# nipponjo/tts-arabic-pytorch

Hardware: AMD Instinct MI355X
Metric: audio samples/sec (FastPitch+HiFi-GAN, synthetic 64-phoneme inputs) (higher is better)
Workload: dtype f32

## Files before the change

### profiles/launch_classes.py

```python
import csv
import re
import sys
from collections import defaultdict


def classes(path):
    d = defaultdict(lambda: [0, 0])
    other = 0
    with open(path) as f:
        for r in csv.DictReader(f):
            dur = int(r['End_Timestamp']) - int(r['Start_Timestamp'])
            m = re.search(r'conv1d_wino4_f32<(\d+), (\d+), (\d+), (\d+), (\d+), (\d+)>', r['Kernel_Name'])
            if not m:
                other += dur
                continue
            k, noct, nst, epi, lp, pt = map(int, m.groups())
            key = (pt, k, lp, 'residual' if epi == 3 else 'plain', int(r['Grid_Size_X']) // int(r['Workgroup_Size_X']))
            d[key][0] += 1
            d[key][1] += dur
    return d, other


a, oa = classes(sys.argv[1])
b, ob = classes(sys.argv[2])
print(f'{"groups":>6} {"k":>3} {"window":>7} {"epilogue":>9} {"blocks":>7} {"calls":>6} {"us parent":>10} {"us tree":>9} {"ratio":>6}')
ta = tb = 0
for key in sorted(set(a) | set(b), key=lambda t: (-t[0], t[1], t[2], t[3], t[4])):
    ca, da = a.get(key, (0, 0))
    cb, db = b.get(key, (0, 0))
    ta += da
    tb += db
    ua, ub = (da / ca / 1e3 if ca else float('nan')), (db / cb / 1e3 if cb else float('nan'))
    print(f'{"seven" if key[0] == 7 else "six":>6} {key[1]:3d} {"vector" if key[2] == 1 else "strip":>7} {key[3]:>9} {key[4]:7d} {max(ca, cb):6d} '
          f'{ua:10.1f} {ub:9.1f} {ub / ua:6.3f}')
print(f'sum over the conv1d_wino4_f32 launches: {ta / 1e6:.2f} -> {tb / 1e6:.2f} ms; every other kernel: {oa / 1e6:.2f} -> {ob / 1e6:.2f} ms (whole trace)')
```

### tts-arabic-pytorch_amd/csrc/common.hpp

```cpp
#pragma once
#include <hip/hip_runtime.h>
#include <stdint.h>
#include <atomic>
#include <cstdarg>
#include <cstdio>
#include <cstdlib>
#include <string>

#include "../../include/ttsamd.h"

namespace ttsamd {

void set_error(const char* fmt, ...);

#define TTS_CHECK_HIP(expr)                                                         \
    do {                                                                            \
        hipError_t e_ = (expr);                                                     \
        if (e_ != hipSuccess) {                                                     \
            ttsamd::set_error("%s failed: %s (%s:%d)", #expr, hipGetErrorString(e_), \
                              __FILE__, __LINE__);                                  \
            return TTSAMD_EHIP;                                                     \
        }                                                                           \
    } while (0)

// ... 25 lines not shown

#define TTS_OPTIONS(X)                                                                                     \
    X(HIFIGAN_STREAMS, 0, 0, 1)    \
    X(WINO, 0, 0, 1)                                              \
    X(WINO2, 0, 0, 31)             \
    X(WINO4, 0, 0, 127)            \
    X(FUSED_PAIR, 0, 0, 1)                   \
    X(FUSED2, 0, 0, 1)                                           \
    X(FUSED2_MASK, 1, 0, 0x1ff)               \
    X(FUSED2_MASK_N1, 1, 0, 0x1ff)          \
    X(FUSED2_WB, 0, 0, 2)                     \
    X(PAIR4, 0, 0, 2)              \
    X(CONVT, 0, 0, 1)                              \
    X(CONVT_WINO, 0, 0, 2)         \
    X(BFO, 0, 0, 1)                \
    X(BFO_CHAIN, 0, 0, 1)                           \
    X(BFO_CHAIN7, 0, 0, 1)                                 \
    X(BFO_FF, 0, 0, 1)                              \
    X(BFO_SPLITK, 0, 0, 1)                                              \
    X(BFO_SMALL_TILES, 0, 0, 1)            \
    X(BF16_ATTN, 0, 0, 1)                                         \
    X(BF16_PACKED_T, 0, 0, 1)                   \
    X(ATT_RA, 0, 1, 4)                             \
    X(ATT_SPLIT, 0, 0, 1)                      \
    X(XCD_W, 0, 0, 1)                            \
    X(XCD_WMAX_KB, 0, 0, 1 << 20)     \
    X(DEEP_SPLITK, 0, 0, 1)        \
    X(TACO_PERSISTENT, 0, 0, 2)    \
    X(TACO_SEG, 0, 8, 1 << 20)     \
    X(RESBLOCK2_PAIR, 1, 0, 0x3f)
enum Opt : int {
#define TTS_OPT_ENUM(name, kind, lo, hi) OPT_##name,
    TTS_OPTIONS(TTS_OPT_ENUM)
#undef TTS_OPT_ENUM
    OPT_COUNT
};
int64_t opt_int(Opt o, int64_t unset);

struct Arena {
    char* base;
    int64_t size;
    int64_t off = 0;
    bool ok = true;
    Arena(void* p, int64_t n) : base((char*)p), size(n) {}
    template <typename T>
    T* take(int64_t count) {
        int64_t bytes = align_up(count * (int64_t)sizeof(T), 256);
        if (base != nullptr && off + bytes > size) ok = false;
        T* r = base ? (T*)(base + off) : nullptr;
        off += bytes;
        return r;
    }
};

struct ConvParams {
    const float* x;
    int64_t x_bs;
    int32_t x_cs;
    const float* w;
    const void* w_bf16;
    const float* w_wino;
    const float* w_wino4;
    int32_t precision;
    const float* bias;
    float* y;
    int64_t y_bs;
    int32_t y_cs, y_ts;
    const float* res;
    int64_t r_bs;
    int32_t r_cs;
    const int64_t* lens_in;
    const int64_t* lens_out;
    int32_t len_in_mul, len_out_mul;
    int32_t Lin, Nout;
    int32_t Cin, Cout, CoutP, K;
    int32_t dil, pad;
    int32_t n_phase;
    int32_t phase_p;
    float in_slope;
    const float* scale;
    int32_t relu_out;
    int32_t mode;
    float div;
    int32_t batch;
    float* splitk_ws;
    int64_t splitk_floats;
    int32_t ksplit;
    int32_t y_packed;
    float pack_slope;
    int32_t x_packed;
    int32_t xcd_w;
    int32_t tile_major;
    int32_t compact;
    unsigned long long* timing;
    const float* w_wino44;
};
constexpr int64_t kSplitKFloats = 4 << 20;
constexpr int64_t kSplitKFloatsFp = 8 << 20;

void conv_log(const char* kind, int K, int cin, int cout, int nout, int batch, int has_res, int mode, int len_mul, int ragged,
              int n_phase);
bool compact_order(const void* lens, int batch);
int32_t launch_conv(const ConvParams& p, hipStream_t stream);
void note_conv_launch(int32_t route, int32_t ksplit);
void last_conv_launch(int32_t* route, int32_t* ksplit);
bool convt_supported(const ConvParams& p);
int32_t launch_convt(const ConvParams& p, hipStream_t stream);
int32_t launch_upsampler(ConvParams& p, const float* x, const float* w, const void* w_bf16, const float* bias, float* y, int cin, int cout,
                         int u, int kt, int L, int len_mul, float in_slope, bool convt_ok, hipStream_t stream, const float* w_wino = nullptr,
                         const float* bias_wino = nullptr);
bool convt_wino_packable(int cin, int cout, int u);
void pack_convt_wino_weight(const float* w, const float* bias, int cin, int cout, int u, float* out_w, float* out_bias);
bool convt_wino_supported(const ConvParams& p, const float* w_wino, const float* bias_wino);
int32_t launch_convt_wino(const ConvParams& p, const float* w_wino, const float* bias_wino, hipStream_t stream);
bool fused_pair_supported(int32_t channels, int32_t k, int32_t dil, int32_t L, const float* x, const float* y);
int32_t launch_fused_pair(int32_t channels, const float* x, float* y, const float* w1, const float* b1, const float* w2,
                          const float* b2, int32_t k, int32_t dil, const int64_t* lens, int32_t len_mul, int32_t L, int32_t batch,
                          int32_t mode, float div, float slope, hipStream_t stream);
bool fused_pair2_supported(int32_t channels, int32_t k, int32_t dil, int32_t L, const float* x, const float* y, int32_t ntw);
int32_t launch_fused_pair2(int32_t channels, const float* x, float* y, const float* w1, const float* b1, const float* w2,
                           const float* b2, int32_t k, int32_t dil, const int64_t* lens, int32_t len_mul, int32_t L, int32_t batch,
                           int32_t mode, float div, float slope, int32_t ntw, hipStream_t stream, const float* w2_wino = nullptr,
                           const float* w1_wino = nullptr);
bool fused_pair4_supported(int32_t channels, int32_t k, int32_t dil, int32_t L, const float* x, const float* y);
int32_t launch_fused_pair4(int32_t channels, const float* x, float* y, const float* w1_wino4, const float* b1, const float* w2_wino4,
                           const float* b2, int32_t k, int32_t dil, const int64_t* lens, int32_t len_mul, int32_t L, int32_t batch,
                           int32_t mode, float div, float slope, hipStream_t stream, int32_t points = 6);
bool resblock2_conv_supported(int32_t channels, int32_t k, int32_t dil, int32_t L, const float* x, const float* y);
int32_t launch_resblock2_conv(int32_t channels, const float* x, float* y, const float* w, const float* b, int32_t k, int32_t dil,
                              const int64_t* lens, int32_t len_mul, int32_t L, int32_t batch, int32_t mode, float div, float slope,
                              hipStream_t stream);
bool resblock2_pair_supported(int32_t channels, int32_t k, int32_t d1, int32_t d2, int32_t L, const float* x, const float* y);
int32_t launch_resblock2_pair(int32_t channels, const float* x, float* y, const float* w1, const float* b1, const float* w2,
                              const float* b2, int32_t k, int32_t d1, int32_t d2, const int64_t* lens, int32_t len_mul, int32_t L,
                              int32_t batch, int32_t mode, float div, float slope, hipStream_t stream);
int wino_route(const ConvParams& p);
int32_t launch_wino(const ConvParams& p, hipStream_t stream);
void pack_wino_weight(const float* w, int cout, int cin, float* out);
int wino2_groups(int k);
int wino2_block_outputs(int coutp, int dil);
int32_t launch_wino2(const ConvParams& p, hipStream_t stream);
void pack_wino2_weight(const float* w, int cout, int cin, int k, float* out);
int wino4_groups(int k);
int wino44_groups(int k);
constexpr int kWino4Default = 127;
bool wino44_wanted(const ConvParams& p);
int wino4_block_outputs(int dil);
int wino4_ksplit(const ConvParams& p);
int32_t launch_splitk_reduce(const ConvParams& q, hipStream_t stream);
int32_t launch_wino4(const ConvParams& p, hipStream_t stream);
void wino4_filter_groups(const float* g, int k, float* o);
void pack_wino4_weight(const float* w, int cout, int cin, int k, float* out);
void wino44_filter_groups(const float* g, int k, float* o);
void pack_wino44_weight(const float* w, int cout, int cin, int k, float* out);
void pack_conv_weight(const float* w, int cout, int cin, int k, float* out);
void pack_convt_weight(const float* w, int cin, int cout, int kt, int u, int p, float* out);
inline int cout_padded(int cout) { return (int)align_up(cout, 32); }
void split_packed_bf16(const float* packed, int64_t n, uint16_t* out);
int32_t default_precision();

#ifdef __HIPCC__
template <int EXTRA = 0>
__device__ __forceinline__ bool live_tile(const int64_t* __restrict__ lens, const int mul, const int n_max, const int tile_w,
                                          const int batch, const unsigned lin, int& b, int& tile) {
    const int lane = threadIdx.x & 63;
    unsigned base = 0;
    for (int u0 = 0; u0 < batch; u0 += 64) {
        int n = 0;
        if constexpr (EXTRA != 0) {
            if (u0 + lane < batch) {
                const int len = (int)lens[u0 + lane] * mul;
                n = (max(min(n_max, len > 0 ? len + EXTRA : 0), 0) + tile_w - 1) / tile_w;
            }
        } else {
            if (u0 + lane < batch) n = (max(min(n_max, (int)lens[u0 + lane] * mul), 0) + tile_w - 1) / tile_w;
        }
        int incl = n;
#pragma unroll
        for (int d = 1; d < 64; d <<= 1) {
            const int t = __shfl_up(incl, d, 64);
            if (lane >= d) incl += t;
        }
        const unsigned total = (unsigned)__shfl(incl, 63, 64);
        if (lin < base + total) {
            const unsigned long long m = __ballot(base + (unsigned)incl > lin);
            const int l = __ffsll((long long)m) - 1;
            b = u0 + l;
            tile = (int)(lin - base) - (__shfl(incl, l, 64) - __shfl(n, l, 64));
            return true;
        }
        base += total;
    }
    return false;
}
#endif

}
```

### tts-arabic-pytorch_amd/csrc/conv_wino4.hip

```cpp
#include <cstdlib>
#include <cstring>

#include <algorithm>
#include <vector>

#include "conv_mfma_common.hpp"
#include "conv_row_epilogue.hpp"
#include "bfo.hpp"

namespace ttsamd {

typedef float w4_f32x4 __attribute__((ext_vector_type(4)));
typedef float w4_f32x2 __attribute__((ext_vector_type(2)));

template <int K, int NOCT_, int NSTAGE_, int PT_ = 6, int LP_ = 1, int CT_ = 0>
struct Wino4Geo {
    static constexpr bool PT7 = PT_ == 7;
    static_assert(PT_ == 6 || (PT7 && (K == 7 || K == 11)), "seven-point groups: k = 7 / 11");
    static_assert(CT_ == 0 || (K == 3 && PT_ == 6 && LP_ == 1), "transposed conv: the k = 3 six-point form at dilation 1");
    static constexpr int WM = 2, WN = 2;
    static constexpr int NSF = K == 1 ? 0 : (K == 3 ? 1 : (K == 7 ? 2 : (PT7 ? 3 : 4)));
    static constexpr int NL = (!PT7 && (K == 7 || K == 1)) ? 1 : 0;
    static constexpr int GSF = PT7 ? 7 : 6;
    static constexpr int SSF = PT7 ? 4 : 3;
// ... 42 lines not shown
    __host__ __device__ static constexpr int sgap(int ph) { return ngap(sph(ph)); }
    static constexpr int JSF = 10;
    __host__ __device__ static constexpr int sflo(int ph) { return glo(ph) / 7; }
    __host__ __device__ static constexpr bool inph(int ph, int g) { return g >= glo(ph) && g < glo(ph) + ngp(ph); }
    __host__ __device__ static constexpr int glast_ph(int ph) { return glo(ph) + ngp(ph) - 1; }
    __host__ __device__ static constexpr int nwj(int ph) {
        return PT7 ? JSF * (glast_ph(ph) / 7 - sflo(ph)) + (glast_ph(ph) % 7 == 0 ? 3 : JSF) : NOCT * ngp(ph);
    }
    static_assert(!PT7 || (NOCT == 1 && glo(0) % 7 <= 1 && glo(NPH - 1) % 7 <= 1 &&
                           (glast_ph(0) % 7 == 0 || glast_ph(0) % 7 >= 5) && glast_ph(NPH - 1) % 7 >= 5),
                  "seven-point phases: start on V0 / V1 of a sub-filter (the partial sums are formed per phase), end on V0 or the last row");
    __host__ __device__ static constexpr int fdiv4(int e) { return e >= 0 ? e / 4 : -((3 - e) / 4); }
    __host__ __device__ static constexpr int vlo(int ph) { return fdiv4(mlo(ph) - (K - 1) / 2); }
    __host__ __device__ static constexpr int nvec(int ph) { return fdiv4(mhi(ph) - (K - 1) / 2) - vlo(ph) + 1; }
    static constexpr int NVP = nvec(0) > nvec(NPH - 1) ? nvec(0) : nvec(NPH - 1);
    __host__ __device__ static constexpr int nljv(int ph) { return NOCT * 2 * nvec(ph); }
    static constexpr int DAV = (K == 3 || K == 1) ? 8 : 16;
    __host__ __device__ static constexpr int tw0v(int ph) { return DAV + 2 * nljv(ph); }
    __host__ __device__ static constexpr int wsv(int ph) { return (sgap(ph) - tw0v(ph)) / nwj(ph); }
    static_assert(LP_ != 1 || (wsv(0) >= 1 && wsv(NPH - 1) >= 1), "one write job per gap at most (vector loads)");
    static constexpr int RAWW = 320;
    static constexpr int NROW = 2 * NOCT;
    static constexpr int RAW_BYTES = 4 * (NROW * RAWW * 4 + 16);
    static constexpr int DAT = K == 7 ? 16 : (K == 11 ? 12 : 8);
    __host__ __device__ static constexpr int nrj(int ph) { return NROW * ((npos(ph) + 1) / 2); }
    __host__ __device__ static constexpr bool loads_in(int ph) { return ph == 0; }
    __host__ __device__ static constexpr int tr_r0(int ph) { return loads_in(ph) ? DAT + 2 * NROW : 0; }
    __host__ __device__ static constexpr int tw0t(int ph) { return tr_r0(ph) + nrj(ph) + 1; }
    __host__ __device__ static constexpr int wst(int ph) { return (sgap(ph) - tw0t(ph)) / nwj(ph); }
    static_assert(LP_ != 2 || (wst(0) >= 1 && wst(NPH - 1) >= 1), "one write job per gap at most (strip path)");
    static constexpr int QX = WSHARE ? 0 : (NOCT * ngq(0)) % PF;
    static constexpr int QMAIN = NOCT * ngq(0) - QX;
    static_assert(QX == 0 || (NPH == 1 && NOCT == 1 && QMAIN >= 2 * PF), "extra queue slots: one phase, one octet");
    static_assert((WSHARE ? NOCT : NOCT * ngq(NPH - 1)) % PF == 0 || QX != 0, "queue slots line up across steps");
    static_assert((size_t)NSTAGE * BUF4 * 16 + (LP_ == 2 ? RAW_BYTES : 0) <= 80 * 1024, "two blocks per CU");
    static_assert(NPH == 1 || NOCT == 1, "phases split an octet's groups");
};

__device__ __host__ constexpr int wino4_tile(int d, int ntup) { return (4 * ntup / (4 * d)) * (4 * d); }

template <int K, int NOCT_, int NSTAGE_, int EPI, int LP, int PT = 6>
__global__ __launch_bounds__(256, kConvMinWaves) void conv1d_wino4_f32(const ConvParams p) {
    extern __shared__ __attribute__((aligned(16))) float4 smem4[];
    constexpr int CTU = EPI == 5 ? 8 : (EPI == 6 ? 2 : 0);
    constexpr bool CT = CTU != 0;
    using G = Wino4Geo<K, NOCT_, NSTAGE_, PT, LP, CTU>;
    constexpr bool PT7 = G::PT7;
    constexpr int WN = G::WN, NSF = G::NSF, NOCT = G::NOCT, NSTAGE = G::NSTAGE, NPL = G::NPL, NGPM = G::NGPM;
    constexpr int CO_BLK = G::CO_BLK, NTUP = G::NTUP, NT_BLK = G::NT_BLK, PF = G::PF;
    constexpr int NPH = G::NPH, NPOSP = G::NPOSP, NM = G::NM;
    constexpr bool D1 = LP == 1, TR = LP == 2;
    static_assert(D1 || TR, "window path");
    const int dil = D1 ? 1 : p.dil;
    const int nt_eff = wino4_tile(dil, NTUP), ntup_eff = nt_eff / 4;
    const int tiles_y = p.CoutP / CO_BLK;
    const int per_tile = tiles_y * p.ksplit;
    const unsigned sidx = blockIdx.x, xcd = sidx & 7u, u = sidx >> 3;
    const int yk = (int)(u % (unsigned)per_tile);
    const unsigned gt = (u / (unsigned)per_tile) * 8u + xcd;
    const int n_tiles_x = (p.Nout + nt_eff - 1) / nt_eff;
    int b = (int)(gt / (unsigned)n_tiles_x);
    int q0 = (int)(gt % (unsigned)n_tiles_x) * nt_eff;
    if (p.compact) {
        int tile = 0;
        if (!live_tile<CT ? 1 : 0>(p.lens_out, p.len_out_mul, p.Nout, nt_eff, p.batch, gt, b, tile)) return;
        b = __builtin_amdgcn_readfirstlane(b);
        q0 = __builtin_amdgcn_readfirstlane(tile) * nt_eff;
    } else if (b >= p.batch) {
        return;
    }
    const int tid = threadIdx.x, lane = tid & 63, wid = tid >> 6;
    const int wm = wid / WN, wn = wid % WN;
    const int ks = yk / tiles_y;
    const int co_blk0 = (yk - ks * tiles_y) * CO_BLK;
    int n_out = p.Nout;
    if constexpr (CT) {
        if (p.lens_out) {
            const int len = min(p.Lin, (int)p.lens_out[b] * p.len_out_mul);
            n_out = len > 0 ? len + 1 : 0;
        }
    } else {
        if (p.lens_out) n_out = min(n_out, (int)p.lens_out[b] * p.len_out_mul);
    }
    if (q0 >= n_out) return;
    int in_len = p.Lin;
    if (p.lens_in) in_len = min(in_len, (int)p.lens_in[b] * p.len_in_mul);

    const int x_cs = p.x_cs, CoutP = p.CoutP;
    const int chunks_all = p.Cin / (8 * NOCT);
    const int c_beg = (int)((int64_t)ks * chunks_all / p.ksplit), n_chunks = (int)((int64_t)(ks + 1) * chunks_all / p.ksplit);
    const int n_groups = (p.Cin / 8) * G::NGW;
    const float* __restrict__ xb = p.x + (int64_t)b * p.x_bs;
    const float in_slope = p.in_slope;

    constexpr bool REG = EPI >= 3, RES = EPI == 3;
    static_assert(!REG || (LP == 1 && K != 1), "register epilogue: dilation 1, k = 3 / 7 / 11");
    static_assert(EPI <= 6 && (!CT || K == 3), "epilogues 0, 3, 4 and the transposed conv's 5 / 6 (k = 3 form)");
    float ep_bias = 0.f;
    if constexpr (!REG) {
        if (tid < CO_BLK && p.bias) ep_bias = p.bias[min(co_blk0 + tid, p.Cout - 1)];
    }

    const int kk = lane >> 5, l31 = lane & 31;
    const int pe = wn * 32 + l31;
    const int col_e = dil == 1 ? 4 * pe : (pe / dil) * 4 * dil + pe % dil;
    f32x16 acc[NPL];
#pragma unroll
    for (int g = 0; g < NPL; ++g)
#pragma unroll
        for (int r = 0; r < 16; ++r) acc[g][r] = 0.f;
    const int ep_row0 = REG ? co_blk0 + __builtin_amdgcn_readfirstlane(wm) * 32 : 0;
    const int ep_voff = (q0 + col_e < n_out ? q0 + col_e : 0) * 4;
    const int ep_rrow = ep_row0 + 4 * kk;
    const bfo_i4 ep_rs = bfo_rsrc(RES ? p.res + (int64_t)b * p.r_bs : nullptr, RES ? (unsigned)p.Cout * (unsigned)p.r_cs * 4u : 0u);
    const bfo_i4 ep_bs = bfo_rsrc(p.bias, (REG && p.bias) ? (unsigned)p.Cout * 4u : 0u);
    w4_f32x4 rq[RES ? 16 : 1], bsq[REG ? 4 : 1];
    constexpr int EP_T0 = RES ? 16 : 0;
#define TTS_EPLOAD_JOB(T)                                                                            \
    {                                                                                                \
        if (RES && (T) < 16)                                                                         \
            rq[RES ? (T) : 0] = __builtin_bit_cast(w4_f32x4, bfo_ld16(ep_rs, ep_voff + (ep_rrow + ((T) & 3) + 8 * ((T) >> 2)) * p.r_cs * 4, 0, 0)); \
        if ((T) >= EP_T0 && (T) < EP_T0 + 4)                                                         \
            bsq[REG ? (T) - EP_T0 : 0] = __builtin_bit_cast(w4_f32x4, bfo_ld16(ep_bs, (ep_rrow + 8 * ((T) - EP_T0)) * 4, 0, 0)); \
    }

    const bfo_i4 wrs = bfo_rsrc(K == 1 ? p.w : (PT7 ? p.w_wino44 : p.w_wino4), (unsigned)n_groups * 2u * (unsigned)CoutP * 16u);
    const int wv = (kk * CoutP + co_blk0 + wm * 32 + l31) * 16;
    const int wstep = 2 * CoutP * 16, wlast = (n_groups - 1) * wstep;
    int wso = c_beg * NOCT * G::NGW * wstep;
    w4_f32x4 aq[PF + G::QX];
    if constexpr (G::QX == 0) {
#pragma unroll
        for (int g = 0; g < PF; ++g) {
            aq[g] = __builtin_bit_cast(w4_f32x4, bfo_ld16(wrs, wv, wso, 0));
            wso = min(wso + wstep, wlast);
        }
    } else {
#pragma unroll
        for (int g = 0; g < PF + G::QX; ++g)
            aq[g] = __builtin_bit_cast(w4_f32x4, bfo_ld16(wrs, wv, min(wso + (g < PF ? g : G::QMAIN + g - PF) * wstep, wlast), 0));
    }

    const int sh = __builtin_amdgcn_readfirstlane((tid >> 7) & 1), skk = __builtin_amdgcn_readfirstlane((tid >> 6) & 1);
    w4_f32x2 sx[D1 ? 1 : NOCT][D1 ? 1 : NPOSP];
    w4_f32x4 sv[D1 ? NOCT : 1][2][D1 ? G::NVP : 1];
    w4_f32x2 ta[NOCT], tb[NOCT];
    w4_f32x2 tf[PT7 ? 5 : 1], te[PT7 ? 4 : 1], td[PT7 ? 3 : 1], th[PT7 ? 2 : 1];
    const int spe = min(lane, ntup_eff - 1);
    const int xw0 = (q0 + 4 * lane) * 4;
    constexpr int pad_c = (K - 1) / 2;
    const int ch_off = (4 * sh + skk) * x_cs;

#define TTS_VJOB_IDX(PH, J)                                                                          \
        const int nv_ = G::nvec(PH);                                                                 \
        const int ol_ = (J) / (2 * nv_), pp_ = ((J) / nv_) % 2, vi_ = (J) % nv_;
#define TTS_VLOAD_JOB(PH, J, XSO)                                                                    \
    {                                                                                                \
        TTS_VJOB_IDX(PH, J)                                                                          \
        const bfo_i4 xrs_ = bfo_rsrc(xb + ((XSO) + ch_off + (8 * ol_ + 2 * pp_) * x_cs), (unsigned)in_len * 4u);     \
        sv[ol_][pp_][vi_] = __builtin_bit_cast(w4_f32x4, bfo_ld16(xrs_, xw0 + 16 * (G::vlo(PH) + vi_), 0, 0));      \
    }
#define TTS_VACT_JOB(PH, A)                                                                          \
    {                                                                                                \
        TTS_VJOB_IDX(PH, (A) / 2)                                                                    \
        if ((A) % 2 == 0) {                                                                          \
            sv[ol_][pp_][vi_].x = bfo_lrelu(sv[ol_][pp_][vi_].x, in_slope);                          \
            sv[ol_][pp_][vi_].y = bfo_lrelu(sv[ol_][pp_][vi_].y, in_slope);                          \
        } else {                                                                                     \
            sv[ol_][pp_][vi_].z = bfo_lrelu(sv[ol_][pp_][vi_].z, in_slope);                          \
            sv[ol_][pp_][vi_].w = bfo_lrelu(sv[ol_][pp_][vi_].w, in_slope);                          \
        }                                                                                            \
    }
    float* const strip = reinterpret_cast<float*>(smem4 + NSTAGE * G::BUF4) + wid * (G::NROW * G::RAWW + 4);
    const int tr_a = (q0 - pad_c * dil) & ~3;
    const int tr_off = q0 + (dil == 1 ? 4 * spe : (spe / dil) * 4 * dil + spe % dil) - pad_c * dil - tr_a;
    w4_f32x4 rv[TR ? G::NROW : 1][2];
#define TTS_TLOAD_JOB(J, XSO)                                                                        \
    {                                                                                                \
        const int pp_ = (J) / 2, vs_ = (J) % 2;                                                      \
        const bfo_i4 xrs_ = bfo_rsrc(xb + ((XSO) + ch_off + (8 * (pp_ / 2) + 2 * (pp_ % 2)) * x_cs), (unsigned)in_len * 4u); \
        const int v_ = lane + 64 * vs_;                                                              \
        rv[pp_][vs_] = __builtin_bit_cast(w4_f32x4, bfo_ld16(xrs_, (vs_ == 1 && lane >= 16) ? BFO_OOB : (tr_a + 4 * v_) * 4, 0, 0)); \
    }
#define TTS_TSTORE_JOB(J)                                                                            \
    {                                                                                                \
        const int pp_ = (J) / 2, vs_ = (J) % 2;                                                      \
        w4_f32x4 a_ = rv[pp_][vs_];                                                                  \
        a_.x = bfo_lrelu(a_.x, in_slope); a_.y = bfo_lrelu(a_.y, in_slope);                          \
        a_.z = bfo_lrelu(a_.z, in_slope); a_.w = bfo_lrelu(a_.w, in_slope);                          \
        const int v_ = lane + 64 * vs_;                                                              \
        float* dst_ = (vs_ == 1 && lane >= 16) ? strip + G::NROW * G::RAWW : strip + pp_ * G::RAWW + 4 * v_;    \
        *reinterpret_cast<w4_f32x4*>(dst_) = a_;                                                     \
    }
// ... 324 lines not shown
        return;
    }
    constexpr int LDS_F = CO_BLK * NT_BLK + CO_BLK;
    static_assert(NT_BLK / 4 == 64, "one wave instruction per row: a lane's columns are the same in every row");
    float* ep = reinterpret_cast<float*>(smem4);
    float* epb = ep + LDS_F - CO_BLK;
    __syncthreads();
    if (tid < CO_BLK) epb[tid] = ep_bias;
#pragma unroll
    for (int r = 0; r < 16; ++r) {
        const int row = wm * 32 + (r & 3) + 8 * (r >> 2) + 4 * kk;
        TTS_OUT_QUAD(r)
        if (pe < ntup_eff) {
            if (dil == 1) {
                *reinterpret_cast<float4*>(ep + row * NT_BLK + col_e) = make_float4(y0, y1, y2, y3);
            } else {
                ep[row * NT_BLK + col_e] = y0;
                ep[row * NT_BLK + col_e + dil] = y1;
                ep[row * NT_BLK + col_e + 2 * dil] = y2;
                ep[row * NT_BLK + col_e + 3 * dil] = y3;
            }
        }
    }
#undef TTS_OUT_QUAD
    __syncthreads();
    const int col = lane * 4, q = q0 + col;
    if (q >= n_out || col >= nt_eff) return;
    if (p.ksplit > 1) {
        constexpr int NR = CO_BLK / 4;
        const bool full = q + 3 < n_out;
        float* __restrict__ pb = p.splitk_ws + ((int64_t)ks * p.batch + b) * Cout * p.Nout;
#pragma unroll 4
        for (int it = 0; it < NR; ++it) {
            const int rl = wid + it * 4;
            const int co = co_blk0 + rl;
            if (co >= Cout) continue;
            const float4 a4 = *reinterpret_cast<const float4*>(ep + rl * NT_BLK + col);
            float* yp = pb + (int64_t)co * p.Nout + q;
            if (full && (p.Nout & 3) == 0) {
                *reinterpret_cast<float4*>(yp) = a4;
            } else {
                const float v[4] = {a4.x, a4.y, a4.z, a4.w};
#pragma unroll
                for (int e = 0; e < 4; ++e)
                    if (q + e < n_out) yp[e] = v[e];
            }
        }
        return;
    }
    conv_row_epilogue<NT_BLK, CO_BLK, K == 1 ? kRowScaleGlobal : kRowScaleNone, K == 1, false, true>(p, ep, epb, K == 1 ? p.scale : nullptr, b,
                                                                                                      co_blk0, CO_BLK, q0, n_out, nt_eff);
}

template <int K, int NOCT, int NSTAGE, int EPI, int LP, int PT = 6>
static int32_t launch_wino4_epi(const ConvParams& p, hipStream_t stream) {
    using G = Wino4Geo<K, NOCT, NSTAGE, PT, LP>;
    constexpr size_t ring = (size_t)G::NSTAGE * G::BUF4 * sizeof(float4);
    constexpr size_t epi = ((size_t)G::CO_BLK * G::NT_BLK + G::CO_BLK) * sizeof(float);
    constexpr size_t strip = LP == 2 ? (size_t)G::RAW_BYTES : 0;
    constexpr size_t lds = (EPI >= 3 || ring + strip > epi) ? ring + strip : epi;
    static_assert(lds <= 80 * 1024, "two blocks per CU");
    static_assert(EPI < 3 || lds == ring, "register epilogue: the ring sets the LDS size");
    static std::atomic<uint64_t> lds_done{0};
    const auto kern = conv1d_wino4_f32<K, NOCT, NSTAGE, EPI, LP, PT>;
    TTS_CHECK_HIP(lds_opt_in((const void*)kern, (int)lds, lds_done));
    const int nt = wino4_tile(p.dil, G::NTUP);
    ConvParams q = p;
    q.ksplit = EPI == 0 ? wino4_ksplit(p) : 1;
    note_conv_launch(PT == 7 ? 4 : 3, q.ksplit);
    const int64_t n_tiles = (int64_t)((p.Nout + nt - 1) / nt) * p.batch;
    const int64_t n_blocks = ((n_tiles + 7) / 8) * 8 * (p.CoutP / G::CO_BLK) * q.ksplit;
    TTS_REQUIRE(n_blocks < ((int64_t)1 << 31), "wino4: %lld blocks", (long long)n_blocks);
    dim3 grid((unsigned)n_blocks, 1, 1);
    q.compact = compact_order(p.lens_out, p.batch) ? 1 : 0;
    hipLaunchKernelGGL(kern, grid, dim3(256), lds, stream, q);
    TTS_CHECK_HIP(hipGetLastError());
    if (q.ksplit > 1) return launch_splitk_reduce(q, stream);
    return 0;
}

template <int K, int NOCT, int NSTAGE>
static int32_t launch_wino4_cfg(const ConvParams& p, hipStream_t stream) {
    if (p.dil == 1) {
        if (wino4_ksplit(p) != 1) return launch_wino4_epi<K, NOCT, NSTAGE, 0, 1>(p, stream);
        if (p.res != nullptr) return launch_wino4_epi<K, NOCT, NSTAGE, 3, 1>(p, stream);
        return launch_wino4_epi<K, NOCT, NSTAGE, 4, 1>(p, stream);
    }
    return launch_wino4_epi<K, NOCT, 2, 0, 2>(p, stream);
}

template <int K>
static int32_t launch_wino44_cfg(const ConvParams& p, hipStream_t stream) {
    if (p.dil == 1) {
        if (wino4_ksplit(p) != 1) return launch_wino4_epi<K, 1, 2, 0, 1, 7>(p, stream);
        if (p.res != nullptr) return launch_wino4_epi<K, 1, 2, 3, 1, 7>(p, stream);
        return launch_wino4_epi<K, 1, 2, 4, 1, 7>(p, stream);
    }
    return launch_wino4_epi<K, 1, 2, 0, 2, 7>(p, stream);
}

bool wino44_wanted(const ConvParams& p) {
    if (p.w_wino44 == nullptr || (p.K != 7 && p.K != 11)) return false;
    return ((int)opt_int(OPT_WINO4, kWino4Default) & (p.K == 7 ? 32 : 64)) != 0;
}

int32_t launch_wino4(const ConvParams& p, hipStream_t stream) {
    if (wino44_wanted(p)) return p.K == 7 ? launch_wino44_cfg<7>(p, stream) : launch_wino44_cfg<11>(p, stream);
    if (p.K == 1) return launch_wino4_epi<1, 4, 2, 0, 1>(p, stream);
    if (p.K == 3) return launch_wino4_cfg<3, 2, 3>(p, stream);
    if (p.K == 7) return launch_wino4_cfg<7, 1, 2>(p, stream);
    if (p.K == 11) return launch_wino4_cfg<11, 1, 3>(p, stream);
    set_error("wino4: kernel size %d not built (1, 3, 7, 11)", p.K);
    return TTSAMD_EINVAL;
}

int wino4_block_outputs(int dil) { return wino4_tile(dil, 64); }

bool convt_wino_packable(int cin, int cout, int u) { return (u == 2 || u == 8) && cin >= 16 && cin % 16 == 0 && cout >= 1 && (u * cout) % 64 == 0; }

bool convt_wino_supported(const ConvParams& p, const float* w_wino, const float* bias_wino) {
    const int u = p.n_phase;
    return w_wino != nullptr && bias_wino != nullptr && p.precision == 0 && convt_wino_packable(p.Cin, p.Cout, u) && p.K == 2 && p.dil == -1 &&
           p.phase_p * 2 == u && p.y_ts == u && p.res == nullptr && p.mode == 0 && p.scale == nullptr && p.relu_out == 0 &&
           !p.x_packed && !p.y_packed && p.in_slope >= 0.f && p.in_slope <= 1.f && p.Lin == p.Nout &&
           (p.x_cs & 3) == 0 && (p.x_bs & 3) == 0 && ((uintptr_t)p.x & 15) == 0 &&
           (p.y_cs & 3) == 0 && (p.y_bs & 3) == 0 && ((uintptr_t)p.y & 15) == 0 &&
           (int64_t)p.Lin * 4 + 64 < ((int64_t)1 << 31) && (int64_t)p.Cout * p.y_cs * 4 < ((int64_t)1 << 31);
}

template <int U>
static int32_t launch_convt_wino_u(const ConvParams& p, const float* w_wino, const float* bias_wino, hipStream_t stream) {
    constexpr int EPI = U == 8 ? 5 : 6;
    using G = Wino4Geo<3, 2, 3, 6, 1, U>;
    constexpr size_t lds = (size_t)G::NSTAGE * G::BUF4 * sizeof(float4);
    static_assert(lds <= 80 * 1024, "two blocks per CU");
    static std::atomic<uint64_t> lds_done{0};
    const auto kern = conv1d_wino4_f32<3, 2, 3, EPI, 1, 6>;
    TTS_CHECK_HIP(lds_opt_in((const void*)kern, (int)lds, lds_done));
    ConvParams q = p;
    q.w_wino4 = w_wino; q.bias = bias_wino;
    q.Cout = U * p.Cout; q.CoutP = q.Cout;
    q.Nout = p.Lin + 1;
    q.K = 3; q.dil = 1; q.pad = 1; q.n_phase = 1; q.ksplit = 1;
    const int64_t n_tiles = (int64_t)((q.Nout + G::NT_BLK - 1) / G::NT_BLK) * p.batch;
    const int64_t n_blocks = ((n_tiles + 7) / 8) * 8 * (q.CoutP / G::CO_BLK);
    TTS_REQUIRE(n_blocks < ((int64_t)1 << 31), "convt wino: %lld blocks", (long long)n_blocks);
    q.compact = compact_order(p.lens_out, p.batch) ? 1 : 0;
    hipLaunchKernelGGL(kern, dim3((unsigned)n_blocks, 1, 1), dim3(256), lds, stream, q);
    TTS_CHECK_HIP(hipGetLastError());
    return 0;
}

int32_t launch_convt_wino(const ConvParams& p, const float* w_wino, const float* bias_wino, hipStream_t stream) {
    TTS_REQUIRE(convt_wino_supported(p, w_wino, bias_wino), "convt wino: unsupported geometry");
    if (p.Nout <= 0) return 0;
    conv_log("convt_wino", 2, p.Cin, p.Cout, p.Nout, p.batch, 0, 0, p.len_out_mul, p.lens_out != nullptr, p.n_phase);
    note_conv_launch(6, 1);
    return p.n_phase == 8 ? launch_convt_wino_u<8>(p, w_wino, bias_wino, stream) : launch_convt_wino_u<2>(p, w_wino, bias_wino, stream);
}

void pack_convt_wino_weight(const float* w, const float* bias, int cin, int cout, int u, float* out_w, float* out_bias) {
    const int rows = u * cout;
    std::vector<float> t((size_t)rows * cin * 3);
    for (int ci = 0; ci < cin; ++ci)
        for (int co = 0; co < cout; ++co)
            for (int j = 0; j < u; ++j) {
                const float* g = w + ((int64_t)ci * cout + co) * 2 * u;
                float* d = t.data() + ((int64_t)(co * u + j) * cin + ci) * 3;
                d[0] = g[j + u]; d[1] = g[j]; d[2] = 0.f;
            }
    pack_wino4_weight(t.data(), rows, cin, 3, out_w);
    for (int r = 0; r < rows; ++r) out_bias[r] = bias ? bias[r / u] : 0.f;
}

int wino4_ksplit(const ConvParams& p) {
    const int bo = wino4_block_outputs(p.dil);
    const int64_t blocks = (int64_t)((p.Nout + bo - 1) / bo) * (p.CoutP / 64) * p.batch;
    constexpr int sk_blocks = 192, sk_target = 224;
    if (blocks >= sk_blocks || p.splitk_ws == nullptr) return 1;
    const int n_chunks = p.Cin / (p.K == 1 ? 32 : (p.K == 3 ? 16 : 8));
    const int64_t per = (int64_t)p.batch * p.Cout * p.Nout;
    int64_t ks = std::min<int64_t>((sk_target + blocks - 1) / blocks, n_chunks / 8);
    ks = std::min<int64_t>(ks, p.splitk_floats / std::max<int64_t>(per, 1));
    return ks >= 2 ? (int)ks : 1;
}

int wino4_groups(int k) { return k == 3 ? 6 : (k == 7 ? 16 : 24); }
int wino44_groups(int k) { return k == 7 ? 13 : (k == 11 ? 20 : 0); }

void wino4_filter_groups(const float* g, int k, float* o) {
    const int nsf = k == 3 ? 1 : (k == 7 ? 2 : 4);
    for (int s = 0; s < nsf; ++s) {
        const double g0 = g[3 * s], g1 = 3 * s + 1 < k ? g[3 * s + 1] : 0.0, g2 = 3 * s + 2 < k ? g[3 * s + 2] : 0.0;
        o[6 * s] = (float)(g0 / 4);
        o[6 * s + 1] = (float)(-(g0 + g1 + g2) / 6);
        o[6 * s + 2] = (float)(-(g0 - g1 + g2) / 6);
        o[6 * s + 3] = (float)(g0 / 24 + g1 / 12 + g2 / 6);
        o[6 * s + 4] = (float)(g0 / 24 - g1 / 12 + g2 / 6);
        o[6 * s + 5] = (float)g2;
    }
// ... 34 lines not shown
```

### tts-arabic-pytorch_amd/csrc/resblock_pair4.hip

```cpp
#include <algorithm>
#include <cstring>

#include "conv_mfma_common.hpp"
#include "bfo.hpp"

namespace ttsamd {

struct FusedPair4Params {
    const float* x;
    float* y;
    const float4* w1;
    const float4* w2;
    const float* b1;
    const float* b2;
    const int64_t* lens;
    int32_t len_mul, L, dil, batch;
    int32_t mode;
    float div, slope;
    int32_t compact;
};

template <int K, int PT_ = 6>
struct Pair4Geo {
    static constexpr bool PT7 = PT_ == 7;
// ... 103 lines not shown
                } else if (sub) {
                    plane = i;
                    if (i == 0) v = 4.f * x[0] + (x[4] - 5.f * x[2]);
                    else if (i == 1) v = (x[4] - 4.f * x[2]) + (x[3] - 4.f * x[1]);
                    else if (i == 2) v = (x[4] - 4.f * x[2]) - (x[3] - 4.f * x[1]);
                    else if (i == 3) v = (x[4] - x[2]) + 2.f * (x[3] - x[1]);
                    else if (i == 4) v = (x[4] - x[2]) - 2.f * (x[3] - x[1]);
                    else v = 4.f * x[1] + (x[5] - 5.f * x[3]);
                } else {
                    plane = i == 0 ? 0 : (i == 1 ? 6 : (i == 2 ? 7 : 5));
                    v = x[i];
                }
                __builtin_amdgcn_sched_barrier(0);
                const float av[4] = {a4.x, a4.y, a4.z, a4.w};
#pragma unroll
                for (int pq = 0; pq < 4; ++pq) acc[plane] = __builtin_amdgcn_mfma_f32_32x32x2f32(av[pq], v[pq], acc[plane], 0, 0, 0);
            }
        }
        if ((UO * NBU) & 1) {
#pragma unroll
            for (int m = 0; m < NX; ++m) xq[0][m] = xq[1][m];
        }
    }
}

template <int PT_, int NPL>
__device__ __forceinline__ void p4_out(const f32x16 (&acc)[NPL], const int r, float (&y)[4]) {
    const float s12 = acc[1][r] + acc[2][r], d12 = acc[1][r] - acc[2][r];
    const float s34 = acc[3][r] + acc[4][r], d34 = acc[3][r] - acc[4][r];
    y[0] = acc[0][r] + s12 + s34;
    y[1] = d12 + 2.f * d34;
    y[2] = s12 + 4.f * s34;
    y[3] = d12 + 8.f * d34 + acc[PT_ == 7 ? 6 : 5][r];
    if constexpr (PT_ == 7) {
        y[0] += acc[5][r];
        y[1] += 0.5f * acc[5][r];
        y[2] += 0.25f * acc[5][r];
        y[3] += 0.125f * acc[5][r];
    } else if constexpr (NPL == 8) {
        y[1] += acc[6][r];
        y[2] += acc[7][r];
    }
}

template <int K, int PT_ = 6>
__global__ __launch_bounds__(256, 2) void resblock_pair4(const FusedPair4Params p) {
    using G = Pair4Geo<K, PT_>;
    constexpr int C = G::C, NOCT = G::NOCT, H = G::H, NPL = G::NPL, NPOS = G::NPOS, PF = G::PF, WQ = G::WQ, ROW = G::ROW;
    extern __shared__ __attribute__((aligned(16))) float4 smem4[];
    const int dil = p.dil, L = p.L;
    const int TS = G::ts(dil);
    const int tid = threadIdx.x, lane = tid & 63, wid = tid >> 6;
    const int kk = lane >> 5, l31 = lane & 31;
    int b = blockIdx.z;
    int q0 = blockIdx.x * TS;
    if (p.compact) {
        int tile = 0;
        if (!live_tile(p.lens, p.len_mul, L, TS, p.batch, blockIdx.z * gridDim.x + blockIdx.x, b, tile)) return;
        b = __builtin_amdgcn_readfirstlane(b);
        q0 = __builtin_amdgcn_readfirstlane(tile) * TS;
    }
    int len = L;
    if (p.lens) len = min(len, (int)p.lens[b] * p.len_mul);
    if (q0 >= len) return;
    const float slope = p.slope;
    const float* __restrict__ xb = p.x + (int64_t)b * C * L;
    float4* Xs = smem4;

    const float4* __restrict__ wl1 = p.w1 + kk * C + l31;
    const float4* __restrict__ wl2 = p.w2 + kk * C + l31;
    float4 aq[PF];
#pragma unroll
    for (int g = 0; g < PF; ++g) aq[g] = wl1[g * 2 * C];

    const int xfirst = q0 - H - H * dil;
    const int xa = xfirst & ~3, off = xfirst - xa;
    {
        const int nv = G::nvec(dil), n_items = 2 * NOCT * nv;
        constexpr int NE = (2 * NOCT * G::WQ + 255) / 256;
        float4 v[NE][4];
#pragma unroll
        for (int u = 0; u < NE; ++u) {
            const int it = tid + 256 * u;
            const int row = min(it / nv, 2 * NOCT - 1), vi = it - row * nv;
            const int ch0 = 8 * (row >> 1) + (row & 1);
            const int voff = it < n_items ? (xa + 4 * vi) * 4 : BFO_OOB;
#pragma unroll
            for (int pq = 0; pq < 4; ++pq) {
                const bfo_i4 rs = bfo_rsrc(xb + (int64_t)(ch0 + 2 * pq) * L, (unsigned)max(len, 0) * 4u);
                v[u][pq] = __builtin_bit_cast(float4, bfo_ld16(rs, voff, 0, 0));
            }
        }
#pragma unroll
        for (int u = 0; u < NE; ++u) {
            const int it = tid + 256 * u;
            if (it < n_items) {
                const int row = it / nv, vi = it - row * nv;
                const float vv[4][4] = {{v[u][0].x, v[u][0].y, v[u][0].z, v[u][0].w}, {v[u][1].x, v[u][1].y, v[u][1].z, v[u][1].w},
                                        {v[u][2].x, v[u][2].y, v[u][2].z, v[u][2].w}, {v[u][3].x, v[u][3].y, v[u][3].z, v[u][3].w}};
#pragma unroll
                for (int j = 0; j < 4; ++j)
                    Xs[row * ROW + j * WQ + vi] = make_float4(p4_lrelu(vv[0][j], slope), p4_lrelu(vv[1][j], slope),
                                                              p4_lrelu(vv[2][j], slope), p4_lrelu(vv[3][j], slope));
            }
        }
    }
    __syncthreads();

    const int jw = wid * 32 + l31;
    const int nqa = G::nqa(dil);
    const int pa = min(jw, nqa - 1);
    const int na = dil == 1 ? 4 * pa : (pa / dil) * 4 * dil + pa % dil;
    f32x16 acc[NPL];
#pragma unroll
    for (int g = 0; g < NPL; ++g)
#pragma unroll
        for (int r = 0; r < 16; ++r) acc[g][r] = 0.f;
    {
        int eo[NPOS];
#pragma unroll
        for (int m = 0; m < NPOS; ++m) {
            const int c = off + na + m * dil;
            eo[m] = (c & 3) * WQ + (c >> 2);
        }
        p4_conv<K, PT_>(acc, aq, Xs + kk * ROW, eo, wl1, wl2);
    }
// ... 126 lines not shown
```

Baseline: 78.16 million.

## Shorten conv kernel prologue: fast division, DPP scan, early weight prefetch

The conv_wino4 and resblock_pair4 prologues now issue weight prefetch loads and the lens load before the live-tile search, so their latency hides behind the index math. The shuffle-based prefix scan becomes a DPP/readlane scan, and the raw length found by the scan is reused instead of reloading lens[b]. Integer divisions for tile mapping use host-precomputed magic multipliers. The aim is to cut per-block startup latency in many small launches, at the cost of extra params and added complexity in the tile-mapping logic.

```diff
diff --git a/profiles/launch_classes.py b/profiles/launch_classes.py
--- a/profiles/launch_classes.py
+++ b/profiles/launch_classes.py
@@ -4,8 +4,12 @@
 from collections import defaultdict
 
 
+pairs = {}
+
+
 def classes(path):
     d = defaultdict(lambda: [0, 0])
+    pr = pairs.setdefault(path, defaultdict(lambda: [0, 0]))
     other = 0
     with open(path) as f:
         for r in csv.DictReader(f):
@@ -13,6 +17,11 @@
             m = re.search(r'conv1d_wino4_f32<(\d+), (\d+), (\d+), (\d+), (\d+), (\d+)>', r['Kernel_Name'])
             if not m:
                 other += dur
+                mp = re.search(r'(resblock_pair[24]<[\d, ]+>)', r['Kernel_Name'])
+                if mp:
+                    e = pr[(mp.group(1), int(r['Grid_Size_X']) // int(r['Workgroup_Size_X']))]
+                    e[0] += 1
+                    e[1] += dur
                 continue
             k, noct, nst, epi, lp, pt = map(int, m.groups())
             key = (pt, k, lp, 'residual' if epi == 3 else 'plain', int(r['Grid_Size_X']) // int(r['Workgroup_Size_X']))
@@ -34,3 +43,10 @@
     print(f'{"seven" if key[0] == 7 else "six":>6} {key[1]:3d} {"vector" if key[2] == 1 else "strip":>7} {key[3]:>9} {key[4]:7d} {max(ca, cb):6d} '
           f'{ua:10.1f} {ub:9.1f} {ub / ua:6.3f}')
 print(f'sum over the conv1d_wino4_f32 launches: {ta / 1e6:.2f} -> {tb / 1e6:.2f} ms; every other kernel: {oa / 1e6:.2f} -> {ob / 1e6:.2f} ms (whole trace)')
+pa, pb = pairs[sys.argv[1]], pairs[sys.argv[2]]
+print(f'\nfused pairs (part of "every other kernel"): {"kernel":>28} {"blocks x":>9} {"calls":>6} {"us parent":>10} {"us tree":>9} {"ratio":>6}')
+for key in sorted(set(pa) | set(pb)):
+    ca, da = pa.get(key, (0, 0))
+    cb, db = pb.get(key, (0, 0))
+    ua, ub = (da / ca / 1e3 if ca else float('nan')), (db / cb / 1e3 if cb else float('nan'))
+    print(f'{"":44}{key[0]:>28} {key[1]:9d} {max(ca, cb):6d} {ua:10.1f} {ub:9.1f} {ub / ua:6.3f}')
diff --git a/tts-arabic-pytorch_amd/csrc/common.hpp b/tts-arabic-pytorch_amd/csrc/common.hpp
--- a/tts-arabic-pytorch_amd/csrc/common.hpp
+++ b/tts-arabic-pytorch_amd/csrc/common.hpp
@@ -101,6 +101,18 @@
         return r;
     }
 };
+
+struct FastDiv {
+    uint32_t mul, shift;
+};
+inline FastDiv fast_div(uint32_t d) {
+    uint32_t l = 0;
+    while (((uint64_t)1 << l) < d) ++l;
+    return FastDiv{(uint32_t)(((((uint64_t)1 << l) - d) << 32) / d) + 1u, l};
+}
+#ifdef __HIPCC__
+__device__ __forceinline__ unsigned fast_div(const unsigned n, const FastDiv f) { return (__umulhi(n, f.mul) + n) >> f.shift; }
+#endif
 
 struct ConvParams {
     const float* x;
@@ -143,6 +155,13 @@
     int32_t compact;
     unsigned long long* timing;
     const float* w_wino44;
+    int32_t lens_same;
+    uint32_t tiles_y;
+    FastDiv per_tile_div;
+    FastDiv tiles_y_div;
+    FastDiv tiles_x_div;
+    uint32_t tiles_x;
+    int32_t tile_w;
 };
 constexpr int64_t kSplitKFloats = 4 << 20;
 constexpr int64_t kSplitKFloatsFp = 8 << 20;
@@ -209,39 +228,57 @@
 int32_t default_precision();
 
 #ifdef __HIPCC__
-template <int EXTRA = 0>
+template <int DPP_CTRL, int ROW_MASK>
+__device__ __forceinline__ int live_tile_scan_step(const int v) {
+    return v + __builtin_amdgcn_update_dpp(0, v, DPP_CTRL, ROW_MASK, 0xf, false);
+}
+__device__ __forceinline__ int live_tile_load(const int64_t* __restrict__ lens, const int batch, const int u0 = 0) {
+    const int lane = threadIdx.x & 63;
+    return u0 + lane < batch ? (int)lens[u0 + lane] : 0;
+}
+template <int EXTRA = 0, bool FIRST_LOADED = true>
 __device__ __forceinline__ bool live_tile(const int64_t* __restrict__ lens, const int mul, const int n_max, const int tile_w,
-                                          const int batch, const unsigned lin, int& b, int& tile) {
+                                          const int batch, const unsigned lin, int& b, int& tile, int& raw_len, const int first) {
     const int lane = threadIdx.x & 63;
     unsigned base = 0;
+    int raw = first;
     for (int u0 = 0; u0 < batch; u0 += 64) {
+        if (!FIRST_LOADED || u0 != 0) raw = live_tile_load(lens, batch, u0);
         int n = 0;
-        if constexpr (EXTRA != 0) {
-            if (u0 + lane < batch) {
-                const int len = (int)lens[u0 + lane] * mul;
+        if (u0 + lane < batch) {
+            const int len = raw * mul;
+            if constexpr (EXTRA != 0) {
                 n = (max(min(n_max, len > 0 ? len + EXTRA : 0), 0) + tile_w - 1) / tile_w;
+            } else {
+                n = (max(min(n_max, len), 0) + tile_w - 1) / tile_w;
             }
-        } else {
-            if (u0 + lane < batch) n = (max(min(n_max, (int)lens[u0 + lane] * mul), 0) + tile_w - 1) / tile_w;
         }
         int incl = n;
-#pragma unroll
-        for (int d = 1; d < 64; d <<= 1) {
-            const int t = __shfl_up(incl, d, 64);
-            if (lane >= d) incl += t;
-        }
-        const unsigned total = (unsigned)__shfl(incl, 63, 64);
+        incl = live_tile_scan_step<0x111, 0xf>(incl);
+        incl = live_tile_scan_step<0x112, 0xf>(incl);
+        incl = live_tile_scan_step<0x114, 0xf>(incl);
+        incl = live_tile_scan_step<0x118, 0xf>(incl);
+        incl = live_tile_scan_step<0x142, 0xa>(incl);
+        incl = live_tile_scan_step<0x143, 0xc>(incl);
+        const unsigned total = (unsigned)__builtin_amdgcn_readlane(incl, 63);
         if (lin < base + total) {
             const unsigned long long m = __ballot(base + (unsigned)incl > lin);
             const int l = __ffsll((long long)m) - 1;
             b = u0 + l;
-            tile = (int)(lin - base) - (__shfl(incl, l, 64) - __shfl(n, l, 64));
+            tile = (int)(lin - base) - (__builtin_amdgcn_readlane(incl, l) - __builtin_amdgcn_readlane(n, l));
+            raw_len = __builtin_amdgcn_readlane(raw, l);
             return true;
         }
         base += total;
     }
     return false;
 }
+template <int EXTRA = 0>
+__device__ __forceinline__ bool live_tile(const int64_t* __restrict__ lens, const int mul, const int n_max, const int tile_w,
+                                          const int batch, const unsigned lin, int& b, int& tile) {
+    int raw_len;
+    return live_tile<EXTRA, false>(lens, mul, n_max, tile_w, batch, lin, b, tile, raw_len, 0);
+}
 #endif
 
 }
diff --git a/tts-arabic-pytorch_amd/csrc/conv_wino4.hip b/tts-arabic-pytorch_amd/csrc/conv_wino4.hip
--- a/tts-arabic-pytorch_amd/csrc/conv_wino4.hip
+++ b/tts-arabic-pytorch_amd/csrc/conv_wino4.hip
@@ -118,44 +118,78 @@
     constexpr bool D1 = LP == 1, TR = LP == 2;
     static_assert(D1 || TR, "window path");
     const int dil = D1 ? 1 : p.dil;
-    const int nt_eff = wino4_tile(dil, NTUP), ntup_eff = nt_eff / 4;
-    const int tiles_y = p.CoutP / CO_BLK;
-    const int per_tile = tiles_y * p.ksplit;
+    const int nt_eff = D1 ? wino4_tile(1, NTUP) : p.tile_w, ntup_eff = nt_eff / 4;
+    const int tid = threadIdx.x, lane = tid & 63, wid = tid >> 6;
+    const int wm = wid / WN, wn = wid % WN;
+    const int kk = lane >> 5, l31 = lane & 31;
+    int lens0 = 0;
+    if (p.compact) lens0 = live_tile_load(p.lens_out, p.batch);
+    const bool split = EPI == 0 && p.ksplit > 1;
+    const unsigned tiles_y = p.tiles_y;
+    const unsigned per_tile = split ? tiles_y * (unsigned)p.ksplit : tiles_y;
     const unsigned sidx = blockIdx.x, xcd = sidx & 7u, u = sidx >> 3;
-    const int yk = (int)(u % (unsigned)per_tile);
-    const unsigned gt = (u / (unsigned)per_tile) * 8u + xcd;
-    const int n_tiles_x = (p.Nout + nt_eff - 1) / nt_eff;
-    int b = (int)(gt / (unsigned)n_tiles_x);
-    int q0 = (int)(gt % (unsigned)n_tiles_x) * nt_eff;
+    const unsigned ut = fast_div(u, p.per_tile_div);
+    const int yk = (int)(u - ut * per_tile);
+    const unsigned gt = ut * 8u + xcd;
+    const int chunks_all = p.Cin / (8 * NOCT);
+    int ks = 0, co_blk0 = yk * CO_BLK, c_beg = 0, n_chunks = chunks_all;
+    if (split) {
+        ks = (int)fast_div((unsigned)yk, p.tiles_y_div);
+        co_blk0 = (yk - ks * (int)tiles_y) * CO_BLK;
+        c_beg = (int)((unsigned)(ks * chunks_all) / (unsigned)p.ksplit);
+        n_chunks = (int)((unsigned)((ks + 1) * chunks_all) / (unsigned)p.ksplit);
+    }
+    const int x_cs = p.x_cs, CoutP = p.CoutP;
+    const int n_groups = (p.Cin / 8) * G::NGW;
+
+    const bfo_i4 wrs = bfo_rsrc(K == 1 ? p.w : (PT7 ? p.w_wino44 : p.w_wino4), (unsigned)n_groups * 2u * (unsigned)CoutP * 16u);
+    const int wv = (kk * CoutP + co_blk0 + wm * 32 + l31) * 16;
+    const int wstep = 2 * CoutP * 16, wlast = (n_groups - 1) * wstep;
+    int wso = c_beg * NOCT * G::NGW * wstep;
+    w4_f32x4 aq[PF + G::QX];
+    if constexpr (G::QX == 0) {
+#pragma unroll
+        for (int g = 0; g < PF; ++g) {
+            aq[g] = __builtin_bit_cast(w4_f32x4, bfo_ld16(wrs, wv, wso, 0));
+            wso = min(wso + wstep, wlast);
+        }
+    } else {
+#pragma unroll
+        for (int g = 0; g < PF + G::QX; ++g)
+            aq[g] = __builtin_bit_cast(w4_f32x4, bfo_ld16(wrs, wv, min(wso + (g < PF ? g : G::QMAIN + g - PF) * wstep, wlast), 0));
+    }
+
+#define TTS_ARG_NOW(V) asm volatile("" ::"s"(V))
+    TTS_ARG_NOW(p.x); TTS_ARG_NOW(p.x_bs); TTS_ARG_NOW(x_cs); TTS_ARG_NOW(p.in_slope);
+    TTS_ARG_NOW(p.Lin); TTS_ARG_NOW(p.Nout); TTS_ARG_NOW(p.len_in_mul); TTS_ARG_NOW(p.len_out_mul);
+    TTS_ARG_NOW(p.lens_in); TTS_ARG_NOW(p.lens_same);
+#undef TTS_ARG_NOW
+    int b, q0, raw_len = 0;
     if (p.compact) {
         int tile = 0;
-        if (!live_tile<CT ? 1 : 0>(p.lens_out, p.len_out_mul, p.Nout, nt_eff, p.batch, gt, b, tile)) return;
+        if (!live_tile<CT ? 1 : 0>(p.lens_out, p.len_out_mul, p.Nout, nt_eff, p.batch, gt, b, tile, raw_len, lens0)) return;
         b = __builtin_amdgcn_readfirstlane(b);
         q0 = __builtin_amdgcn_readfirstlane(tile) * nt_eff;
-    } else if (b >= p.batch) {
-        return;
-    }
-    const int tid = threadIdx.x, lane = tid & 63, wid = tid >> 6;
-    const int wm = wid / WN, wn = wid % WN;
-    const int ks = yk / tiles_y;
-    const int co_blk0 = (yk - ks * tiles_y) * CO_BLK;
+        raw_len = __builtin_amdgcn_readfirstlane(raw_len);
+    } else {
+        b = (int)fast_div(gt, p.tiles_x_div);
+        q0 = (int)(gt - (unsigned)b * p.tiles_x) * nt_eff;
+        if (b >= p.batch) return;
+        if (p.lens_out) raw_len = __builtin_amdgcn_readfirstlane((int)p.lens_out[b]);
+    }
     int n_out = p.Nout;
     if constexpr (CT) {
         if (p.lens_out) {
-            const int len = min(p.Lin, (int)p.lens_out[b] * p.len_out_mul);
+            const int len = min(p.Lin, raw_len * p.len_out_mul);
             n_out = len > 0 ? len + 1 : 0;
         }
     } else {
-        if (p.lens_out) n_out = min(n_out, (int)p.lens_out[b] * p.len_out_mul);
+        if (p.lens_out) n_out = min(n_out, raw_len * p.len_out_mul);
     }
     if (q0 >= n_out) return;
     int in_len = p.Lin;
-    if (p.lens_in) in_len = min(in_len, (int)p.lens_in[b] * p.len_in_mul);
-
-    const int x_cs = p.x_cs, CoutP = p.CoutP;
-    const int chunks_all = p.Cin / (8 * NOCT);
-    const int c_beg = (int)((int64_t)ks * chunks_all / p.ksplit), n_chunks = (int)((int64_t)(ks + 1) * chunks_all / p.ksplit);
-    const int n_groups = (p.Cin / 8) * G::NGW;
+    if (p.lens_in) in_len = min(in_len, (p.lens_same ? raw_len : __builtin_amdgcn_readfirstlane((int)p.lens_in[b])) * p.len_in_mul);
+
     const float* __restrict__ xb = p.x + (int64_t)b * p.x_bs;
     const float in_slope = p.in_slope;
 
@@ -167,7 +201,6 @@
         if (tid < CO_BLK && p.bias) ep_bias = p.bias[min(co_blk0 + tid, p.Cout - 1)];
     }
 
-    const int kk = lane >> 5, l31 = lane & 31;
     const int pe = wn * 32 + l31;
     const int col_e = dil == 1 ? 4 * pe : (pe / dil) * 4 * dil + pe % dil;
     f32x16 acc[NPL];
@@ -188,23 +221,6 @@
             rq[RES ? (T) : 0] = __builtin_bit_cast(w4_f32x4, bfo_ld16(ep_rs, ep_voff + (ep_rrow + ((T) & 3) + 8 * ((T) >> 2)) * p.r_cs * 4, 0, 0)); \
         if ((T) >= EP_T0 && (T) < EP_T0 + 4)                                                         \
             bsq[REG ? (T) - EP_T0 : 0] = __builtin_bit_cast(w4_f32x4, bfo_ld16(ep_bs, (ep_rrow + 8 * ((T) - EP_T0)) * 4, 0, 0)); \
-    }
-
-    const bfo_i4 wrs = bfo_rsrc(K == 1 ? p.w : (PT7 ? p.w_wino44 : p.w_wino4), (unsigned)n_groups * 2u * (unsigned)CoutP * 16u);
-    const int wv = (kk * CoutP + co_blk0 + wm * 32 + l31) * 16;
-    const int wstep = 2 * CoutP * 16, wlast = (n_groups - 1) * wstep;
-    int wso = c_beg * NOCT * G::NGW * wstep;
-    w4_f32x4 aq[PF + G::QX];
-    if constexpr (G::QX == 0) {
-#pragma unroll
-        for (int g = 0; g < PF; ++g) {
-            aq[g] = __builtin_bit_cast(w4_f32x4, bfo_ld16(wrs, wv, wso, 0));
-            wso = min(wso + wstep, wlast);
-        }
-    } else {
-#pragma unroll
-        for (int g = 0; g < PF + G::QX; ++g)
-            aq[g] = __builtin_bit_cast(w4_f32x4, bfo_ld16(wrs, wv, min(wso + (g < PF ? g : G::QMAIN + g - PF) * wstep, wlast), 0));
     }
 
     const int sh = __builtin_amdgcn_readfirstlane((tid >> 7) & 1), skk = __builtin_amdgcn_readfirstlane((tid >> 6) & 1);
@@ -635,6 +651,16 @@
                                                                                                       co_blk0, CO_BLK, q0, n_out, nt_eff);
 }
 
+static void set_wino4_tile_map(ConvParams& q, int tile_w, int co_blk) {
+    q.tile_w = tile_w;
+    q.tiles_y = (uint32_t)(q.CoutP / co_blk);
+    q.tiles_x = (uint32_t)((q.Nout + tile_w - 1) / tile_w);
+    q.per_tile_div = fast_div(q.tiles_y * (uint32_t)q.ksplit);
+    q.tiles_y_div = fast_div(q.tiles_y);
+    q.tiles_x_div = fast_div(q.tiles_x);
+    q.lens_same = q.lens_in == q.lens_out ? 1 : 0;
+}
+
 template <int K, int NOCT, int NSTAGE, int EPI, int LP, int PT = 6>
 static int32_t launch_wino4_epi(const ConvParams& p, hipStream_t stream) {
     using G = Wino4Geo<K, NOCT, NSTAGE, PT, LP>;
@@ -656,6 +682,7 @@
     TTS_REQUIRE(n_blocks < ((int64_t)1 << 31), "wino4: %lld blocks", (long long)n_blocks);
     dim3 grid((unsigned)n_blocks, 1, 1);
     q.compact = compact_order(p.lens_out, p.batch) ? 1 : 0;
+    set_wino4_tile_map(q, nt, G::CO_BLK);
     hipLaunchKernelGGL(kern, grid, dim3(256), lds, stream, q);
     TTS_CHECK_HIP(hipGetLastError());
     if (q.ksplit > 1) return launch_splitk_reduce(q, stream);
@@ -729,6 +756,7 @@
     const int64_t n_blocks = ((n_tiles + 7) / 8) * 8 * (q.CoutP / G::CO_BLK);
     TTS_REQUIRE(n_blocks < ((int64_t)1 << 31), "convt wino: %lld blocks", (long long)n_blocks);
     q.compact = compact_order(p.lens_out, p.batch) ? 1 : 0;
+    set_wino4_tile_map(q, G::NT_BLK, G::CO_BLK);
     hipLaunchKernelGGL(kern, dim3((unsigned)n_blocks, 1, 1), dim3(256), lds, stream, q);
     TTS_CHECK_HIP(hipGetLastError());
     return 0;
diff --git a/tts-arabic-pytorch_amd/csrc/resblock_pair4.hip b/tts-arabic-pytorch_amd/csrc/resblock_pair4.hip
--- a/tts-arabic-pytorch_amd/csrc/resblock_pair4.hip
+++ b/tts-arabic-pytorch_amd/csrc/resblock_pair4.hip
@@ -179,26 +179,30 @@
     const int TS = G::ts(dil);
     const int tid = threadIdx.x, lane = tid & 63, wid = tid >> 6;
     const int kk = lane >> 5, l31 = lane & 31;
+    int lens0 = 0;
+    if (p.compact) lens0 = live_tile_load(p.lens, p.batch);
+    const float4* __restrict__ wl1 = p.w1 + kk * C + l31;
+    const float4* __restrict__ wl2 = p.w2 + kk * C + l31;
+    float4 aq[PF];
+#pragma unroll
+    for (int g = 0; g < PF; ++g) aq[g] = wl1[g * 2 * C];
+
     int b = blockIdx.z;
     int q0 = blockIdx.x * TS;
+    int len = L;
     if (p.compact) {
-        int tile = 0;
-        if (!live_tile(p.lens, p.len_mul, L, TS, p.batch, blockIdx.z * gridDim.x + blockIdx.x, b, tile)) return;
+        int tile = 0, raw_len = 0;
+        if (!live_tile(p.lens, p.len_mul, L, TS, p.batch, blockIdx.z * gridDim.x + blockIdx.x, b, tile, raw_len, lens0)) return;
         b = __builtin_amdgcn_readfirstlane(b);
         q0 = __builtin_amdgcn_readfirstlane(tile) * TS;
-    }
-    int len = L;
-    if (p.lens) len = min(len, (int)p.lens[b] * p.len_mul);
+        len = min(len, __builtin_amdgcn_readfirstlane(raw_len) * p.len_mul);
+    } else if (p.lens) {
+        len = min(len, (int)p.lens[b] * p.len_mul);
+    }
     if (q0 >= len) return;
     const float slope = p.slope;
     const float* __restrict__ xb = p.x + (int64_t)b * C * L;
     float4* Xs = smem4;
-
-    const float4* __restrict__ wl1 = p.w1 + kk * C + l31;
-    const float4* __restrict__ wl2 = p.w2 + kk * C + l31;
-    float4 aq[PF];
-#pragma unroll
-    for (int g = 0; g < PF; ++g) aq[g] = wl1[g * 2 * C];
 
     const int xfirst = q0 - H - H * dil;
     const int xa = xfirst & ~3, off = xfirst - xa;
```

New measurement: 78.55 million, median of 6. Within noise of the previous version (+0.5%).
